# google/nerfactor

Hardware: AMD Instinct MI355X
Metric: rays/sec (NeRF coarse+fine render, 64+128 samples/ray) (higher is better)
Workload: dtype bf16; 1 GPU; lego_3072-shaped NeRF coarse+fine MLP render, 800x800 rays/view, 64+128 samples (BASELINE.json configs[1]); rays_per_view=640000, n_samples_coarse=64, n_samples_fine=128, kernel_variant=7

## Files before the change

### include/nfx.h

```cpp
#ifndef NFX_H_
#define NFX_H_

#include <stddef.h>
#include <stdint.h>

#ifdef __cplusplus
extern "C" {
#endif

#if defined(__GNUC__)
#define NFX_API __attribute__((visibility("default")))
#else
#define NFX_API
#endif

#define NFX_OK 0
#define NFX_EINVAL (-1)
#define NFX_EALIGN (-2)
#define NFX_EHIP (-3)
#define NFX_ENOSUP (-4)

#define NFX_PREC_BF16 0
#define NFX_PREC_FP32 1
#define NFX_PREC_FP32_NATIVE 2
// ... 199 lines not shown
    float *ga, *gb;
    int d;
    float w;
    int kind;
    int flags;
} nfx_loss_term;
NFX_API int nfx_pair_loss_fwd(const nfx_loss_term *terms, int n_terms, const float *dev_alpha, float bg, int64_t n,
                      float *dev_loss, void *stream);
NFX_API int nfx_pair_loss_bwd(const nfx_loss_term *terms, int n_terms, const float *dev_alpha, float bg, int64_t n,
                      const float *dev_dloss, void *stream);


NFX_API int nfx_nerf_sigma_fwd(const float *dev_rayo, const float *dev_rayd, const float *dev_z, int64_t n_rays,
                       int n_samples, const void *dev_geom_blob, int prec, float *dev_sigma, void *stream);

NFX_API size_t nfx_nerf_geom_packed_bytes(int prec);
NFX_API int nfx_nerf_pack_geom_weights(const float *const kernels[12], const float *const biases[12], int prec,
                               void *blob, size_t blob_bytes);
NFX_API int nfx_nerf_sigma_grad(const float *dev_rayo, const float *dev_rayd, const float *dev_z, int64_t n_rays,
                        int n_samples, const void *dev_geom_blob, int prec, float *dev_normal_sigma,
                        void *stream);

NFX_API size_t nfx_nerf_sigma_grad_workspace_bytes(int64_t n_rays, int n_samples);
NFX_API int nfx_nerf_sigma_grad_rows(const float *dev_rayo, const float *dev_rayd, const float *dev_z, int64_t n_rays,
                             int n_samples, const void *dev_geom_blob, int prec, float *dev_normal_sigma,
                             void *dev_workspace, size_t workspace_bytes, void *stream);

NFX_API int nfx_nerf_refine_select(const float *dev_rgbs, const float *dev_z, const float *dev_rayd, int64_t n_rays,
                           int n_samples, float t_min, float a_lo, float a_hi, float sigma_margin, int dilate,
                           int *dev_list, int *dev_count, void *stream);
NFX_API int nfx_nerf_sigma_refine(const float *dev_rayo, const float *dev_rayd, const float *dev_z, int64_t n_rays,
                          int n_samples, const void *dev_geom_blob_fp32, const int *dev_list, const int *dev_count,
                          float *dev_rgbs, void *stream);

#define NFX_OCCGRID_MAX_RES 1024
#define NFX_OCCGRID_MAX_PROBES (1ll << 30)
NFX_API int nfx_nerf_sigma_fwd_list(const float *dev_rayo, const float *dev_rayd, const float *dev_z, int64_t n_rays,
                            int n_samples, const void *dev_geom_blob, int prec, const int *dev_list,
                            const int *dev_count, float *dev_sigma, void *stream);
NFX_API size_t nfx_occgrid_workspace_bytes(int64_t n_rays, int n_samples);
NFX_API int nfx_occgrid_select(const float *dev_rayo, const float *dev_rayd, const float *dev_z, int64_t n_rays,
                       int n_samples, const uint32_t *dev_bits, int res, const float *box, const float *bbox,
                       float *dev_sigma, void *dev_workspace, size_t workspace_bytes, void *stream);
NFX_API int nfx_occgrid_bake(const float *dev_probe_sigma, int res, int probes, float margin, int dilate,
                     uint32_t *dev_bits, uint32_t *dev_workspace, void *stream);


NFX_API int nfx_selftest_mfma_bf16(const float *dev_a, const float *dev_b, float *dev_d, void *stream);
NFX_API int nfx_mlp_generic_split_hilo(void *dev_blob, int d_in, int n_layers, const int *widths, const int *skip_input,
                                       int train, void *stream);
NFX_API size_t nfx_mlp_generic_packed_bytes(int d_in, int n_layers, const int *widths, const int *skip_input, int prec);
NFX_API int nfx_mlp_generic_pack(const float *const *kernels, const float *const *biases, int d_in, int n_layers,
                                 const int *widths, const int *skip_input, int prec, void *blob, size_t blob_bytes);
NFX_API int nfx_mlp_generic_fwd(const float *dev_x, int64_t n, int ld_x, int d_in, int n_layers, const int *widths,
                                const int *acts, const int *skip_input, const void *dev_blob, int prec, float *dev_y,
                                int ld_y, int col0, void *stream);
NFX_API size_t nfx_mlp_generic_train_packed_bytes(int d_in, int n_layers, const int *widths, const int *skip_input,
                                                  int prec);
NFX_API int nfx_mlp_generic_pack_train(const float *const *kernels, const float *const *biases, int d_in, int n_layers,
                                       const int *widths, const int *skip_input, int prec, void *blob,
                                       size_t blob_bytes);
NFX_API size_t nfx_mlp_generic_bwd_workspace_bytes(int64_t n, int d_in, int n_layers, const int *widths,
                                                   const int *skip_input, int prec);
NFX_API int nfx_mlp_generic_bwd(const float *dev_x, int64_t n, int ld_x, int d_in, int n_layers, const int *widths,
                                const int *acts, const int *skip_input, const void *dev_train_blob, int prec,
                                const float *dev_dy, int ld_dy, int col0_dy, float *dev_dx, int ld_dx,
// ... 15 lines not shown
```

### nerfactor_amd/_capi.py

```python
import ctypes
import os

import torch

_HERE = os.path.dirname(os.path.abspath(__file__))
LIB_PATH = os.path.join(_HERE, 'libnfx.so')
if os.environ.get('NFX_LIB_PATH'):
    LIB_PATH = os.environ['NFX_LIB_PATH']

PREC_BF16, PREC_FP32, PREC_FP32_NATIVE = 0, 1, 2
ACT_NONE, ACT_RELU, ACT_SIGMOID, ACT_SOFTPLUS = 0, 1, 2, 3
IN_XYZ, IN_XYZ_LDIR, IN_Z_RUSINK = 0, 1, 2

if not os.path.exists(LIB_PATH):
    raise ImportError(
        "%s not found: build it with `python -m nerfactor_amd.build` (or __graft_entry__.build()); "
        "nerfactor_amd has no fallback path." % LIB_PATH)

lib = ctypes.CDLL(LIB_PATH)

_p = ctypes.c_void_p
_i = ctypes.c_int
_i64 = ctypes.c_int64
_f = ctypes.c_float
# ... 38 lines not shown
    'nfx_composite_bwd': (_i, [_p, _p, _p, _p, _i64, _i, _i, _p, _p, _p]),
    'nfx_nerf_train_packed_bytes': (_sz, [_i]),
    'nfx_nerf_pack_train_weights': (_i, [_pp, _pp, _i, _p, _sz]),
    'nfx_nerf_bwd_workspace_bytes': (_sz, [_i64, _i]),
    'nfx_nerf_mlp_bwd': (_i, [_p, _p, _p, _i64, _i, _p, _i, _p, _p, _sz, _pp, _pp, _p]),
    'nfx_brdf_train_packed_bytes': (_sz, []),
    'nfx_brdf_pack_train_weights': (_i, [_pp, _pp, _i, _i, _p, _sz]),
    'nfx_brdf_spec_bwd_workspace_bytes': (_sz, [_i, _i64]),
    'nfx_brdf_spec_bwd': (_i, [_p, _p, _p, _p, _i, _p, _i, _p, _i, _i64, _p, _p, _p, _p, _sz, _p]),
    'nfx_brdf_spec_bwd_list_bytes': (_sz, [_i64, _i]),
    'nfx_brdf_spec_bwd_rows': (_i, [_p, _p, _p, _p, _i, _p, _i, _p, _i, _i64, _p, _p, _p, _p, _sz, _p, _sz, _p]),
    'nfx_brdf_rows_fwd': (_i, [_p, _i, _p, _i64, _i, _p, _i, _p, _p]),
    'nfx_brdf_rows_bwd_workspace_bytes': (_sz, [_i, _i64, _i]),
    'nfx_brdf_rows_bwd': (_i, [_p, _i, _p, _i64, _i, _p, _i, _p, _p, _sz, _p, _pp, _pp, _p]),
    'nfx_shade_bwd_workspace_bytes': (_sz, [_i]),
    'nfx_shade_bwd': (_i, [_p, _p, _p, _p, _p, _p, _f, _f, _p, _p, _p, _p, _i64, _i, _i, _p, _p, _p, _p, _p, _p,
                           _p, _p, _sz, _p]),
    'nfx_l2_normalize_rows': (_i, [_p, _p, _i64, _i, _f, _p]),
    'nfx_l2_normalize_rows_bwd': (_i, [_p, _p, _p, _i64, _i, _f, _p]),
    'nfx_light_smoothness': (_i, [_p, _i, _i, _f, _f, _p, _p, _p]),
    'nfx_pair_loss_fwd': (_i, [_p, _i, _p, _f, _i64, _p, _p]),
    'nfx_pair_loss_bwd': (_i, [_p, _i, _p, _f, _i64, _p, _p]),
    'nfx_pack_gather': (_i, [_p, _p, _i64, _p, _p]),
    'nfx_amsgrad_step': (_i, [_p, _p, _p, _p, _p, _i64, _f, _f, _f, _f, _i64, _p]),
    'nfx_amsgrad_step_size': (_f, [_f, _f, _f, _i64]),
    'nfx_amsgrad_step_dev': (_i, [_p, _p, _p, _p, _p, _i64, _p, _f, _f, _f, _p]),
    'nfx_nerf_sigma_fwd': (_i, [_p, _p, _p, _i64, _i, _p, _i, _p, _p]),
    'nfx_lvis_fwd_rows': (_i, [_p, _p, _i64, _f, _p, _i, _p, _i, _p, _sz, _p, _p, _p, _p]),
    'nfx_zero_rows': (_i, [_p, _p, _i64, _i, _p]),
    'nfx_shade_fwd_rows': (_i, [_p, _p, _p, _p, _p, _p, _f, _f, _p, _p, _p, _p, _p, _i64, _i, _i, _i, _p, _p]),
    'nfx_shade_olat_fwd_rows': (_i, [_p, _p, _p, _p, _p, _p, _f, _f, _p, _p, _p, _p, _f, _f, _i64, _i, _i, _p, _p, _p, _p]),
    'nfx_nerf_refine_select': (_i, [_p, _p, _p, _i64, _i, _f, _f, _f, _f, _i, _p, _p, _p]),
    'nfx_nerf_sigma_refine': (_i, [_p, _p, _p, _i64, _i, _p, _p, _p, _p, _p]),
    'nfx_nerf_sigma_fwd_list': (_i, [_p, _p, _p, _i64, _i, _p, _i, _p, _p, _p, _p]),
    'nfx_occgrid_workspace_bytes': (_sz, [_i64, _i]),
    'nfx_occgrid_select': (_i, [_p, _p, _p, _i64, _i, _p, _i, _p, _p, _p, _p, _sz, _p]),
    'nfx_occgrid_bake': (_i, [_p, _i, _i, _f, _i, _p, _p, _p]),
    'nfx_nerf_geom_packed_bytes': (_sz, [_i]),
    'nfx_nerf_pack_geom_weights': (_i, [_pp, _pp, _i, _p, _sz]),
    'nfx_nerf_sigma_grad': (_i, [_p, _p, _p, _i64, _i, _p, _i, _p, _p]),
    'nfx_nerf_sigma_grad_workspace_bytes': (_sz, [_i64, _i]),
    'nfx_nerf_sigma_grad_rows': (_i, [_p, _p, _p, _i64, _i, _p, _i, _p, _p, _sz, _p]),
    'nfx_selftest_mfma_bf16': (_i, [_p, _p, _p, _p]),
    'nfx_selftest_sincos': (_i, [_p, _i64, _i, _p, _p]),
    'nfx_selftest_tr16': (_i, [_p, _p, _p, _i, _p]),
    'nfx_mlp_generic_packed_bytes': (_sz, [_i, _i, _p, _p, _i]),
    'nfx_mlp_generic_pack': (_i, [_pp, _pp, _i, _i, _p, _p, _i, _p, _sz]),
    'nfx_mlp_generic_fwd': (_i, [_p, _i64, _i, _i, _i, _p, _p, _p, _p, _i, _p, _i, _i, _p]),
    'nfx_mlp_generic_train_packed_bytes': (_sz, [_i, _i, _p, _p, _i]),
    'nfx_mlp_generic_pack_train': (_i, [_pp, _pp, _i, _i, _p, _p, _i, _p, _sz]),
    'nfx_mlp_generic_bwd_workspace_bytes': (_sz, [_i64, _i, _i, _p, _p, _i]),
    'nfx_mlp_generic_split_hilo': (_i, [_p, _i, _i, _p, _p, _i, _p]),
    'nfx_brdf_rows_geom_fwd': (_i, [_p, _p, _p, _p, _i, _p, _i, _i64, _i, _p, _i, _p, _p]),
    'nfx_brdf_rows_geom_bwd': (_i, [_p, _p, _p, _i, _p, _i, _i64, _i, _p, _i, _p, _p, _p]),
    'nfx_embed_bwd': (_i, [_p, _i64, _i, _i, _p, _i, _i, _p, _p]),
    'nfx_mlp_generic_bwd': (_i, [_p, _i64, _i, _i, _i, _p, _p, _p, _p, _i, _p, _i, _i, _p, _i, _pp, _pp, _p, _sz, _p]),
    'nfx_embed': (_i, [_p, _p, _p, _i64, _i, _i, _i, _i, _p, _i, _i, _p]),
}

for _name, (_res, _args) in SIGNATURES.items():
    _fn = getattr(lib, _name)
    _fn.restype = _res
    _fn.argtypes = _args


class NfxError(RuntimeError):
    """Raised for any non-zero return of the C-ABI; mirrors how the reference surfaces failures as
    Python exceptions (tf.errors.InvalidArgumentError from tf.debugging.*)."""


def last_error():
    buf = ctypes.create_string_buffer(512)
    lib.nfx_last_error(buf, 512)
    return buf.value.decode()


def check(rc, what):
    if rc != 0:
        raise NfxError("%s failed (%d): %s" % (what, rc, last_error()))


OPTION_KEYS = ('nerf_variant', 'nerf_fold', 'nerf_blocks', 'm128_blocks', 'lvis_variant', 'brdf_variant', 'brdf_ct', 'nerf_bwd',
               'nerf_bwd_nw', 'm128_bwd', 'wgrad_lds', 'wgrad_slabs', 'wgrad_rounds', 'wgrad_narrow', 'wgrad_fused', 'lvis_verify', 'lvis_rows', 'brdf_bwd_rows', 'nerf_bwd_rows', 'sigma_grad_rows', 'sigma_variant')


def set_option(key, value):
    check(lib.nfx_set_option(key.encode(), int(value)), 'nfx_set_option(%s)' % key)


def unset_option(key):
    check(lib.nfx_unset_option(key.encode()), 'nfx_unset_option(%s)' % key)


def get_option(key):
    v, isset = _i(0), _i(0)
    check(lib.nfx_get_option(key.encode(), ctypes.byref(v), ctypes.byref(isset)), 'nfx_get_option(%s)' % key)
    return v.value if isset.value else None


class option:

    def __init__(self, key, value):
        self.key, self.value = key, value

    def __enter__(self):
        self.prev = get_option(self.key)
        if self.value is None:
            unset_option(self.key)
        else:
            set_option(self.key, self.value)
        return self

    def __exit__(self, *exc):
        if self.prev is None:
            unset_option(self.key)
        else:
# ... 9 lines not shown
```

### nerfactor_amd/build.py

```python
import fcntl
import os
import subprocess
import sys
from concurrent.futures import ThreadPoolExecutor

HERE = os.path.dirname(os.path.abspath(__file__))
ROOT = os.path.dirname(HERE)
CSRC = os.path.join(HERE, 'csrc')
OBJDIR = os.path.join(ROOT, 'build', 'obj')
LIB = os.path.join(HERE, 'libnfx.so')

HIPCC = os.environ.get('HIPCC', '/opt/rocm/bin/hipcc')
FLAGS = ['--offload-arch=gfx950', '-O3', '-std=c++17', '-ffp-contract=off', '-fPIC', '-fvisibility=hidden',
         '-Wno-unused-result', '-I' + os.path.join(ROOT, 'include')]


VGPR_FORM = ['-mllvm', '-amdgpu-mfma-vgpr-form']
FAST_DIV = ['-fno-hip-fp32-correctly-rounded-divide-sqrt']
PER_FILE_FLAGS = {'lvis_v2.hip': VGPR_FORM, 'nerf_mlp.hip': VGPR_FORM, 'nerf_mlp_v6.hip': VGPR_FORM, 'nerf_sigma_v6.hip': VGPR_FORM,
                  'nerf_geom.hip': VGPR_FORM, 'mlp128_bwd_fused.hip': VGPR_FORM, 'shade.hip': FAST_DIV}


def _sources():
    return sorted(f for f in os.listdir(CSRC) if f.endswith(('.hip', '.cpp')))


def _headers_mtime():
    hs = [os.path.join(CSRC, f) for f in os.listdir(CSRC) if f.endswith('.hpp')]
    hs.append(os.path.join(ROOT, 'include', 'nfx.h'))
    return max(os.path.getmtime(h) for h in hs)


def _job(src, force):
    obj = os.path.join(OBJDIR, src + '.o')
    spath = os.path.join(CSRC, src)
    newest = max(os.path.getmtime(spath), _headers_mtime())
    for line in open(spath):
        if line.startswith('#include "') and line.rstrip().endswith('.hip"'):
            newest = max(newest, os.path.getmtime(os.path.join(CSRC, line.split('"')[1])))
    cmd = [HIPCC] + FLAGS + PER_FILE_FLAGS.get(src, []) + ['-x', 'hip', '-c', spath, '-o', obj]
    stamp = obj + '.cmd'
    same_cmd = os.path.exists(stamp) and open(stamp).read() == ' '.join(cmd)
    return src, obj, cmd, force or not (same_cmd and os.path.exists(obj) and os.path.getmtime(obj) >= newest)


def _compile(job, verbose):
    src, obj, cmd, stale = job
    if not stale:
        return obj, False
    if verbose:
        print(' '.join(cmd), flush=True)
    res = subprocess.run(cmd, stdout=subprocess.PIPE, stderr=subprocess.STDOUT, text=True)
# ... 46 lines not shown
```

### nerfactor_amd/csrc/capi.cpp

```cpp
#include <hip/hip_runtime.h>
#include <stdarg.h>
#include <stdio.h>
#include <stdlib.h>
#include <string.h>

#include <atomic>
#include <vector>

#include "../../include/nfx.h"
#include "nerf_layout.hpp"
#include "nerf_fold_layout.hpp"
#include "pack.hpp"

static thread_local char g_err[512] = "";

int nfx_fail(int code, const char* fmt, ...) {
    va_list ap;
    va_start(ap, fmt);
    vsnprintf(g_err, sizeof(g_err), fmt, ap);
    va_end(ap);
    return code;
}
#define fail nfx_fail
int nfx_hip_result(int e, const char* what);
// ... 27 lines not shown
                         float*, float*, float*, float*, float*, hipStream_t);
int nfx_launch_sample_fine(const float*, const float*, long long, int, int, const float*, float*,
                           hipStream_t);
int nfx_launch_surface(const float*, const float*, const float*, const float*, long long, int, float, int, float*, float*,
                       float*, float*, hipStream_t);
int nfx_launch_selftest_mfma(const float*, const float*, float*, hipStream_t);
int nfx_launch_selftest_sincos(const float*, long long, int, float*, hipStream_t);

int nfx_version(void) { return 100; }

int nfx_last_error(char* buf, size_t len) {
    if (!buf || len == 0) return NFX_EINVAL;
    strncpy(buf, g_err, len - 1);
    buf[len - 1] = 0;
    return NFX_OK;
}

namespace {
struct Option {
    const char* key;
    std::atomic<int> value;
    std::atomic<int> is_set;
};
Option g_options[] = {
    {"nerf_variant", {0}, {0}},
    {"nerf_fold", {0}, {0}},
    {"nerf_blocks", {0}, {0}},
    {"m128_blocks", {0}, {0}},
    {"lvis_variant", {0}, {0}},
    {"lvis_verify", {0}, {0}},
    {"lvis_rows", {0}, {0}},
    {"brdf_bwd_rows", {0}, {0}},
    {"sigma_variant", {0}, {0}},
    {"sigma_grad_rows", {0}, {0}},
    {"nerf_bwd_rows", {0}, {0}},
    {"brdf_variant", {0}, {0}},
    {"brdf_ct", {0}, {0}},
    {"nerf_bwd", {0}, {0}},
    {"nerf_bwd_nw", {0}, {0}},
    {"m128_bwd", {0}, {0}},
    {"wgrad_lds", {0}, {0}},
    {"wgrad_slabs", {0}, {0}},
    {"wgrad_rounds", {0}, {0}},
    {"wgrad_narrow", {0}, {0}},
    {"wgrad_fused", {0}, {0}},
    {"wgrad_splits", {0}, {0}},
    {"wgrad_map", {0}, {0}},
};
Option* find_option(const char* key) {
    if (!key) return nullptr;
    for (Option& o : g_options)
        if (strcmp(o.key, key) == 0) return &o;
    return nullptr;
}
}

int nfx_option_int(const char* key, int dflt) {
    Option* o = find_option(key);
    return o && o->is_set.load(std::memory_order_acquire) ? o->value.load(std::memory_order_relaxed) : dflt;
}
int nfx_set_option(const char* key, int value) {
    Option* o = find_option(key);
    if (!o) return fail(NFX_EINVAL, "nfx_set_option: unknown option '%s'", key ? key : "(null)");
    o->value.store(value, std::memory_order_relaxed);
    o->is_set.store(1, std::memory_order_release);
    return NFX_OK;
// ... 254 lines not shown
```

### nerfactor_amd/csrc/capi_geom.cpp

```cpp
#include <hip/hip_runtime.h>
#include <math.h>
#include <string.h>

#include <vector>

#include "../../include/nfx.h"
#include "nerf_geom_layout.hpp"
#include "pack.hpp"

int nfx_fail(int code, const char* fmt, ...);
int nfx_hip_result(int e, const char* what);
extern "C" int nfx_option_int(const char* name, int dflt);

#define REQUIRE(cond, ...) \
    do {                   \
        if (!(cond)) return nfx_fail(NFX_EINVAL, __VA_ARGS__); \
    } while (0)
#define ALIGNED(p, a) ((((uintptr_t)(p)) & ((a)-1)) == 0)

extern "C" {
int nfx_launch_nerf_sigma_geo(const float*, const float*, const float*, long long, int, const void*, float*, int,
                              hipStream_t);
int nfx_launch_nerf_sigma_grad(const float*, const float*, const float*, long long, int, const void*, float*, int,
                               hipStream_t);
int nfx_launch_refine_select(const float*, const float*, const float*, long long, int, float, float, float, float, int, int*, int*,
                             hipStream_t);
int nfx_launch_nerf_sigma_v6(const float*, const float*, const float*, long long, int, const void*, float*, int, hipStream_t);
int nfx_launch_nerf_sigma_grad_list(const float*, const float*, const float*, long long, int, const void*, float*, const int*,
                                    const int*, int, hipStream_t);
int nfx_launch_nerf_sigma_grad_x3_list(const float*, const float*, const float*, long long, int, const void*, float*,
                                       const int*, const int*, int, hipStream_t);
int nfx_launch_select_density(const float*, long long, float*, void*, hipStream_t);
size_t nfx_nerf_bwd_list_bytes(long long n_pts);
int nfx_launch_nerf_sigma_x3_list(const float*, const float*, const float*, long long, int, const void*, float*, const int*,
                                  const int*, int, hipStream_t);
int nfx_launch_nerf_sigma_x3(const float*, const float*, const float*, long long, int, const void*, float*, int,
                             hipStream_t);
int nfx_launch_nerf_sigma_grad_x3(const float*, const float*, const float*, long long, int, const void*, float*, int,
                                  hipStream_t);
int nfx_launch_nerf_sigma_v6_list(const float*, const float*, const float*, long long, int, const void*, float*, const int*,
                                  const int*, int, hipStream_t);
int nfx_launch_nerf_sigma_x3_list_flat(const float*, const float*, const float*, long long, int, const void*, float*,
                                       const int*, const int*, int, hipStream_t);
size_t nfx_occgrid_list_bytes(long long n_pts);
int nfx_launch_occgrid_select(const float*, const float*, const float*, long long, int, const uint32_t*, int, const float*,
                              const float*, float*, void*, hipStream_t);
int nfx_launch_occgrid_bake(const float*, int, int, float, int, uint32_t*, uint32_t*, hipStream_t);

size_t nfx_nerf_geom_packed_bytes(int prec) {
    using namespace nfx::nerf;
    if (prec == NFX_PREC_BF16) return (size_t)kGeoBlobBytes;
    if (prec == NFX_PREC_FP32) return 2 * (size_t)kGeoWeightBytes + kGeoFloats * sizeof(float);
    return 0;
}
}

static int pack_geom_half(const float* const kernels[12], const float* const biases[12], uint8_t* w0, float* fl) {
    using namespace nfx;
    using namespace nfx::pack;
    std::vector<uint8_t> fwd(nfx_nerf_packed_bytes(NFX_PREC_BF16));
    int rc = nfx_nerf_pack_weights(kernels, biases, NFX_PREC_BF16, fwd.data(), fwd.size());
    if (rc) return rc;
    const size_t enc_bytes = (size_t)nerf::chunk_frag_offset(64) * 1024;
    memcpy(w0, fwd.data(), enc_bytes);
    memcpy(w0 + enc_bytes, fwd.data() + (size_t)nerf::chunk_frag_offset(72) * 1024, 16 * 1024);
    uint8_t* w = w0 + enc_bytes + 16 * 1024;
    std::vector<float> sink(256);
    const Seg hid256{kHidden, 256, 0, nullptr};
    auto hidden_t = [](const float* k) {
        std::vector<float> t((size_t)256 * 256);
        for (int r = 0; r < 256; ++r)
            for (int c = 0; c < 256; ++c) t[(size_t)c * 256 + r] = k[(size_t)r * 256 + c];
        return t;
    };
    auto input_t = [](const float* k, int row0) {
        std::vector<float> t((size_t)256 * 64, 0.f);
// ... 80 lines not shown
        return nfx_hip_result(nfx_launch_nerf_sigma_x3(rayo, rayd, z, (long long)n_rays * n_samples, n_samples, blob,
                                                       sigma, nfx_option_int("nerf_blocks", 256), (hipStream_t)stream),
                              "nerf_sigma_fwd(fp32)");
    return nfx_hip_result(launch_sigma_bf16(rayo, rayd, z, (long long)n_rays * n_samples, n_samples, blob, sigma,
                                            (hipStream_t)stream),
                          "nerf_sigma_fwd");
}

int nfx_nerf_refine_select(const float* rgbs, const float* z, const float* rayd, int64_t n_rays, int n_samples,
                           float t_min, float a_lo, float a_hi, float sigma_margin, int dilate, int* list, int* count,
                           void* stream) {
    REQUIRE(n_rays >= 0 && n_samples >= 1 && n_samples <= 512, "nfx_nerf_refine_select: bad shape (1 <= S <= 512, got %d)", n_samples);
    REQUIRE(n_rays * (int64_t)n_samples < (int64_t)1 << 31, "nfx_nerf_refine_select: %lld samples do not fit int32 indices",
            (long long)(n_rays * n_samples));
    REQUIRE(dilate >= 0 && dilate <= 8, "nfx_nerf_refine_select: dilate = %d (0 .. 8)", dilate);
    REQUIRE(count, "nfx_nerf_refine_select: null count");
    if (n_rays > 0) REQUIRE(rgbs && z && rayd && list, "nfx_nerf_refine_select: null pointer");
    if (n_rays > 0 && !ALIGNED(rgbs, 16)) return nfx_fail(NFX_EALIGN, "nfx_nerf_refine_select: rgbs must be 16-byte aligned");
    return nfx_hip_result(nfx_launch_refine_select(rgbs, z, rayd, (long long)n_rays, n_samples, t_min, a_lo, a_hi, sigma_margin, dilate,
                                                   list, count, (hipStream_t)stream), "nerf_refine_select");
}

int nfx_nerf_sigma_refine(const float* rayo, const float* rayd, const float* z, int64_t n_rays, int n_samples,
                          const void* blob, const int* list, const int* count, float* rgbs, void* stream) {
    REQUIRE(n_rays >= 0 && n_samples >= 1, "nfx_nerf_sigma_refine: bad shape");
    if (n_rays == 0) return NFX_OK;
    REQUIRE(rayo && rayd && z && blob && list && count && rgbs, "nfx_nerf_sigma_refine: null pointer");
    if (!ALIGNED(blob, 16)) return nfx_fail(NFX_EALIGN, "nfx_nerf_sigma_refine: blob must be 16-byte aligned");
    return nfx_hip_result(nfx_launch_nerf_sigma_x3_list(rayo, rayd, z, (long long)n_rays * n_samples, n_samples, blob, rgbs,
                                                        list, count, nfx_option_int("nerf_blocks", 256),
                                                        (hipStream_t)stream), "nerf_sigma_refine");
}

int nfx_nerf_sigma_grad(const float* rayo, const float* rayd, const float* z, int64_t n_rays, int n_samples,
                        const void* geom_blob, int prec, float* normal_sigma, void* stream) {
    REQUIRE(n_rays >= 0 && n_samples >= 1, "nfx_nerf_sigma_grad: bad shape");
    REQUIRE(prec == NFX_PREC_BF16 || prec == NFX_PREC_FP32, "nfx_nerf_sigma_grad: bad prec %d", prec);
    if (n_rays == 0) return NFX_OK;
    REQUIRE(rayo && rayd && z && geom_blob && normal_sigma, "nfx_nerf_sigma_grad: null pointer");
    if (!ALIGNED(geom_blob, 16) || !ALIGNED(normal_sigma, 16))
        return nfx_fail(NFX_EALIGN, "nfx_nerf_sigma_grad: blob and output must be 16-byte aligned");
    if (prec == NFX_PREC_FP32)
        return nfx_hip_result(nfx_launch_nerf_sigma_grad_x3(rayo, rayd, z, (long long)n_rays * n_samples, n_samples,
                                                            geom_blob, normal_sigma,
                                                            nfx_option_int("nerf_blocks", 256), (hipStream_t)stream),
                              "nerf_sigma_grad(fp32)");
    return nfx_hip_result(nfx_launch_nerf_sigma_grad(rayo, rayd, z, (long long)n_rays * n_samples, n_samples,
                                                     geom_blob, normal_sigma, nfx_option_int("nerf_blocks", 256),
                                                     (hipStream_t)stream),
                          "nerf_sigma_grad");
}

static size_t sigma_grad_sigma_bytes(long long n_pts) { return ((size_t)n_pts * 4 + 15) / 16 * 16; }
size_t nfx_nerf_sigma_grad_workspace_bytes(int64_t n_rays, int n_samples) {
    if (n_rays <= 0 || n_samples <= 0) return 0;
    const long long n_pts = (long long)n_rays * n_samples;
    return sigma_grad_sigma_bytes(n_pts) + nfx_nerf_bwd_list_bytes(n_pts);
}

int nfx_nerf_sigma_grad_rows(const float* rayo, const float* rayd, const float* z, int64_t n_rays, int n_samples,
                             const void* geom_blob, int prec, float* normal_sigma, void* workspace,
                             size_t workspace_bytes, void* stream) {
    REQUIRE(n_rays >= 0 && n_samples >= 1, "nfx_nerf_sigma_grad_rows: bad shape");
    REQUIRE(prec == NFX_PREC_BF16 || prec == NFX_PREC_FP32, "nfx_nerf_sigma_grad_rows: bad prec %d", prec);
    if (n_rays == 0) return NFX_OK;
    REQUIRE(rayo && rayd && z && geom_blob && normal_sigma && workspace, "nfx_nerf_sigma_grad_rows: null pointer");
// ... 89 lines not shown
```

### nerfactor_amd/csrc/nerf_geom_x3.hip

```cpp
#include "feat_store.hpp"
#include "mlp_x3.hpp"
#include "nerf_geom_layout.hpp"

namespace nfx {
namespace geo3 {

using x3::Pair;
constexpr int kNW = x3::kNW;
constexpr int kRows = kNW * 32;
constexpr int kZeroTile = nerf::kGeoFloats;
constexpr int kLds = 2 * x3::kSlot + (nerf::kGeoFloats + 32) * 4;
constexpr int kNLD = 4;

template <int KS1, int KS2, int NL_SELF, int NL_NEXT, int KS1A, int KS2A>
__device__ __forceinline__ void fwd_layer(x3::Stream& st, int tid, const float* bias, const Pair (&b1)[KS1A],
                                          const Pair (&b2)[KS2A], Pair (&bout)[16], unsigned (&m)[4]) {
    static_for<0, 8>([&](auto T) {
        constexpr int t = decltype(T)::value;
        f32x16 acc;
        x3::tile<KS1, KS2, (t == 7 ? NL_NEXT : NL_SELF)>(st, tid, bias + 32 * t, b1, b2, acc);
        const unsigned bits = bwd::relu_bits16(acc);
        if constexpr (t & 1) m[t >> 1] |= bits << 16;
        else m[t >> 1] = bits;
        x3::acc_to_pair<true>(acc, bout[2 * t], bout[2 * t + 1]);
    });
}

__device__ __forceinline__ void put(Pair (&dst)[16], int t, int r, float v) {
    __bf16 a, b;
    x3::split(v, a, b);
    dst[2 * t + (r >> 3)].hi[r & 7] = a;
    dst[2 * t + (r >> 3)].lo[r & 7] = b;
}

__device__ __forceinline__ void dgrad(x3::Stream& st, int tid, const float* zero, const Pair (&dz)[16],
                                      const unsigned (&m)[4], Pair (&dout)[16]) {
    static_for<0, 8>([&](auto T) {
        constexpr int t = decltype(T)::value;
        f32x16 acc;
        x3::tile<16, 0, kNLD>(st, tid, zero, dz, dz, acc);
#pragma unroll
        for (int r = 0; r < 16; ++r) put(dout, t, r, bwd::mask_bit(m, t, r) ? acc[r] : 0.f);
    });
}

template <int NL_LAST>
__device__ __forceinline__ void input_grad(x3::Stream& st, int tid, const float* zero, const Pair (&dz)[16],
                                           f32x16 (&dpe)[2]) {
    static_for<0, 2>([&](auto T) {
        constexpr int t = decltype(T)::value;
        f32x16 acc;
        x3::tile<16, 0, (t == 1 ? NL_LAST : kNLD)>(st, tid, zero, dz, dz, acc);
#pragma unroll
        for (int r = 0; r < 16; ++r) dpe[t][r] += acc[r];
    });
}

template <bool GRAD>
__global__ __launch_bounds__(kNW * 64, 1) void nerf_sigma_x3_kernel(
    const float* __restrict__ rayo, const float* __restrict__ rayd, const float* __restrict__ zbuf, long long n_pts,
    int n_samples, const char* __restrict__ blob, float* __restrict__ out, const int* __restrict__ list,
    const int* __restrict__ count, int list_stride) {
    extern __shared__ __attribute__((aligned(16))) char smem[];
    using namespace nerf;
    if (list != nullptr) {
        n_pts = *count;
        if ((long long)blockIdx.x * kRows >= n_pts) return;
    }
    const int tid = threadIdx.x, lane = tid & 63, wave = tid >> 6, h = lane >> 5, p = lane & 31;
    float* fl = reinterpret_cast<float*>(smem + 2 * x3::kSlot);
    {
        const float* src = reinterpret_cast<const float*>(blob + 2 * (size_t)kGeoWeightBytes);
        for (int i = tid; i < kGeoFloats; i += kNW * 64) fl[i] = src[i];
        if (tid < 32) fl[kZeroTile + tid] = 0.f;
    }
    const float* zero = fl + kZeroTile;
    x3::Stream st;
    st.base = reinterpret_cast<const u32x4*>(blob);
    st.end = reinterpret_cast<const u32x4*>(blob + (GRAD ? (size_t)kGeoWeightBytes : (size_t)kGeoFwdFrags * kFragBytes));
    st.ghi = st.base;
    st.lo_off = kGeoWeightBytes / 16;
    st.ring = smem;
    x3::prologue<kNL0>(st, tid);
    const long long n_tiles = (n_pts + kRows - 1) / kRows;
    for (long long tile = blockIdx.x; tile < n_tiles; tile += gridDim.x) {
        const long long row = tile * kRows + wave * 32 + p;
        const bool valid = row < n_pts;
        long long mm = valid ? row : n_pts - 1;
        if (list != nullptr) mm = list[mm];
        float x[3];
        {
            const long long ray = mm / n_samples;
            const float zz = zbuf[mm];
#pragma unroll
            for (int k = 0; k < 3; ++k) x[k] = rayo[ray * 3 + k] + rayd[ray * 3 + k] * zz;
        }
        Pair pe[4];
        x3::posenc_pair<10>(x, h, pe);
        unsigned mk[8][4];
        Pair ha[16], hb[16];
        fwd_layer<4, 0, kNL0, kNLH>(st, tid, fl + 256 * 0, pe, pe, ha, mk[0]);
        fwd_layer<16, 0, kNLH, kNLH>(st, tid, fl + 256 * 1, ha, pe, hb, mk[1]);
        fwd_layer<16, 0, kNLH, kNLH>(st, tid, fl + 256 * 2, hb, pe, ha, mk[2]);
        fwd_layer<16, 0, kNLH, kNLH>(st, tid, fl + 256 * 3, ha, pe, hb, mk[3]);
        fwd_layer<16, 0, kNLH, kNL5>(st, tid, fl + 256 * 4, hb, pe, ha, mk[4]);
        fwd_layer<16, 4, kNL5, kNLH>(st, tid, fl + 256 * 5, ha, pe, hb, mk[5]);
        fwd_layer<16, 0, kNLH, kNLH>(st, tid, fl + 256 * 6, hb, pe, ha, mk[6]);
        fwd_layer<16, 0, kNLH, kNLH>(st, tid, fl + 256 * 7, ha, pe, hb, mk[7]);
        float sigma;
        {
            f32x16 acc;
            x3::tile<16, 0, (GRAD ? kNLD : kNL0)>(st, tid, fl + kGeoBiasSig, hb, pe, acc);
            sigma = acc[0];
        }
        if constexpr (!GRAD) {
            if (valid && h == 0) {
                if (list != nullptr) out[list_stride * (mm + 1) - 1] = sigma;
                else out[row] = sigma;
            }
        } else {
#pragma unroll
            for (int t = 0; t < 8; ++t)
#pragma unroll
                for (int r = 0; r < 16; ++r) {
                    const float wv = fl[kGeoWSig + 32 * t + (r & 3) + 8 * (r >> 2) + 4 * h];
                    put(ha, t, r, bwd::mask_bit(mk[7], t, r) ? wv : 0.f);
                }
            f32x16 dpe[2];
#pragma unroll
            for (int t = 0; t < 2; ++t)
#pragma unroll
                for (int r = 0; r < 16; ++r) dpe[t][r] = 0.f;
            dgrad(st, tid, zero, ha, mk[6], hb);
            dgrad(st, tid, zero, hb, mk[5], ha);
            input_grad<kNLD>(st, tid, zero, ha, dpe);
            dgrad(st, tid, zero, ha, mk[4], hb);
            dgrad(st, tid, zero, hb, mk[3], ha);
            dgrad(st, tid, zero, ha, mk[2], hb);
            dgrad(st, tid, zero, hb, mk[1], ha);
            dgrad(st, tid, zero, ha, mk[0], hb);
            input_grad<kNL0>(st, tid, zero, hb, dpe);
            float g[3] = {0.f, 0.f, 0.f};
#pragma unroll
            for (int q = 0; q < 32; ++q) {
                const float dq = dpe[q >> 4][q & 15];
                if (q < 30) {
                    const float freq = (float)(1 << (q / 3));
                    const float other = sin_shifted(x[q % 3] * freq, h ^ 1);
                    g[q % 3] += dq * freq * (h ? -other : other);
                } else if (q == 30) {
                    if (h) g[2] += dq; else g[0] += dq;
                } else {
                    if (!h) g[1] += dq;
                }
            }
#pragma unroll
            for (int k = 0; k < 3; ++k) g[k] += __shfl_xor(g[k], 32, 64);
            if (valid && h == 0) {
                const float on = sigma > 0.f ? 1.f : 0.f;
                const float gx = g[0] * on, gy = g[1] * on, gz = g[2] * on;
                const float inv = -1.0f / sqrtf(fmaxf(gx * gx + gy * gy + gz * gz, 1e-12f));
                reinterpret_cast<float4*>(out)[list != nullptr ? mm : row] = make_float4(gx * inv, gy * inv, gz * inv, sigma);
            }
        }
    }
}

template <bool GRAD>
static int launch(const float* rayo, const float* rayd, const float* z, long long n_pts, int n_samples,
                  const void* blob, float* out, int max_blocks, hipStream_t st, const int* list = nullptr,
                  const int* count = nullptr, int list_stride = 4) {
    if (n_pts <= 0) return 0;
    const long long tiles = (n_pts + kRows - 1) / kRows;
    const int grid = (int)(tiles < max_blocks ? tiles : max_blocks);
    auto k = nerf_sigma_x3_kernel<GRAD>;
    hipError_t e = hipFuncSetAttribute(reinterpret_cast<const void*>(k), hipFuncAttributeMaxDynamicSharedMemorySize, kLds);
    if (e != hipSuccess) return (int)e;
    hipLaunchKernelGGL(k, dim3(grid), dim3(kNW * 64), kLds, st, rayo, rayd, z, n_pts, n_samples, (const char*)blob, out,
                       list, count, list_stride);
    return (int)hipGetLastError();
}

}
}

extern "C" int nfx_launch_nerf_sigma_grad_x3(const float* rayo, const float* rayd, const float* z, long long n_pts,
                                             int n_samples, const void* blob, float* out, int max_blocks,
                                             hipStream_t st) {
    return nfx::geo3::launch<true>(rayo, rayd, z, n_pts, n_samples, blob, out, max_blocks, st);
}
extern "C" int nfx_launch_nerf_sigma_x3(const float* rayo, const float* rayd, const float* z, long long n_pts,
                                        int n_samples, const void* blob, float* out, int max_blocks, hipStream_t st) {
    return nfx::geo3::launch<false>(rayo, rayd, z, n_pts, n_samples, blob, out, max_blocks, st);
}
extern "C" int nfx_launch_nerf_sigma_grad_x3_list(const float* rayo, const float* rayd, const float* z, long long n_pts,
                                                  int n_samples, const void* blob, float* out, const int* list,
                                                  const int* count, int max_blocks, hipStream_t st) {
    return nfx::geo3::launch<true>(rayo, rayd, z, n_pts, n_samples, blob, out, max_blocks, st, list, count);
}
extern "C" int nfx_launch_nerf_sigma_x3_list(const float* rayo, const float* rayd, const float* z, long long n_pts,
                                             int n_samples, const void* blob, float* rgbs, const int* list,
                                             const int* count, int max_blocks, hipStream_t st) {
    return nfx::geo3::launch<false>(rayo, rayd, z, n_pts, n_samples, blob, rgbs, max_blocks, st, list, count);
}
extern "C" int nfx_launch_nerf_sigma_x3_list_flat(const float* rayo, const float* rayd, const float* z, long long n_pts,
                                                  int n_samples, const void* blob, float* out, const int* list,
                                                  const int* count, int max_blocks, hipStream_t st) {
    return nfx::geo3::launch<false>(rayo, rayd, z, n_pts, n_samples, blob, out, max_blocks, st, list, count, 1);
}
```

### nerfactor_amd/ops.py

```python
import ctypes
import os

import numpy as np
import torch

from . import _capi
from ._capi import PREC_BF16, PREC_FP32, PREC_FP32_NATIVE, check, lib

_PREC = {'bf16': PREC_BF16, 'fp32': PREC_FP32, 'fp32_native': PREC_FP32_NATIVE, PREC_BF16: PREC_BF16, PREC_FP32: PREC_FP32,
         PREC_FP32_NATIVE: PREC_FP32_NATIVE}
_ACT = {None: 0, 'none': 0, 'relu': 1, 'sigmoid': 2, 'softplus': 3}


def _ptr(t):
    return None if t is None else ctypes.c_void_p(t.data_ptr())


def _stream():
    return ctypes.c_void_p(torch.cuda.current_stream().cuda_stream)


def _dev(t, name, shape=None):
    if t is None:
        return None
# ... 793 lines not shown
            first = ws_bytes // 4 - nerf_bwd_list_words((hi - lo) * s)[3]
            NERF_BWD_STATS.append((ws.view(torch.int32)[first:first + 1].clone(), (hi - lo) * s))
    return ws


def pack_nerf_geom_weights(kernels, biases, prec='bf16'):
    if len(kernels) != 12 or len(biases) != 12:
        raise _capi.NfxError("pack_nerf_geom_weights: need 12 kernels and 12 biases")
    return _pack(lib.nfx_nerf_geom_packed_bytes, lib.nfx_nerf_pack_geom_weights, kernels, biases, (_PREC[prec],))


def _ray_args(rayo, rayd, z, blob):
    rayo = _dev(rayo, 'rayo', (None, 3))
    n = rayo.shape[0]
    rayd = _dev(rayd, 'rayd', (n, 3))
    z = _dev(z, 'z', (n, None))
    if not blob.is_cuda or blob.dtype != torch.uint8:
        raise _capi.NfxError("blob must be a CUDA uint8 tensor")
    return rayo, rayd, z, n, z.shape[1]


def nerf_sigma_fwd(rayo, rayd, z, blob, prec='bf16'):
    rayo, rayd, z, n, s = _ray_args(rayo, rayd, z, blob)
    out = torch.empty((n, s), dtype=torch.float32, device=z.device)
    check(lib.nfx_nerf_sigma_fwd(_ptr(rayo), _ptr(rayd), _ptr(z), n, s, _ptr(blob), _PREC[prec], _ptr(out),
                                 _stream()), 'nfx_nerf_sigma_fwd')
    return out


def nerf_refine_last_sample(rayo, rayd, z, rgbs, geom_blob_fp32):
    n, s = z.shape
    if n == 0 or s < 2:
        return rgbs
    sig = nerf_sigma_fwd(rayo, rayd, z[:, -1:].contiguous(), geom_blob_fp32, 'fp32')
    rgbs[:, -1, 3] = sig[:, 0]
    return rgbs


REFINE_T_MIN, REFINE_A_LO, REFINE_A_HI, REFINE_DILATE = 1e-3, 1e-3, 0.999, 0
REFINE_MARGIN_FACTOR = 2.


def nerf_refine_coarse(rayo, rayd, z, rgbs, geom_blob_fp32, t_min=REFINE_T_MIN, a_lo=REFINE_A_LO, a_hi=REFINE_A_HI,
                       dilate=REFINE_DILATE, sigma_margin=0., want_count=False):
    rayo, rayd, z, n, s = _ray_args(rayo, rayd, z, geom_blob_fp32)
    if not (isinstance(rgbs, torch.Tensor) and rgbs.is_contiguous()):
        raise _capi.NfxError("nerf_refine_coarse: rgbs is updated in place and must be contiguous")
    rgbs = _dev(rgbs, 'rgbs', (n, s, 4))
    count = torch.empty(1, dtype=torch.int32, device=z.device)
    if n == 0 or s < 2:
        count.zero_()
        return (rgbs, count) if want_count else rgbs
    lst = torch.empty(n * s, dtype=torch.int32, device=z.device)
    check(lib.nfx_nerf_refine_select(_ptr(rgbs), _ptr(z), _ptr(rayd), n, s, t_min, a_lo, a_hi, sigma_margin, dilate, _ptr(lst), _ptr(count),
                                     _stream()), 'nfx_nerf_refine_select')
    check(lib.nfx_nerf_sigma_refine(_ptr(rayo), _ptr(rayd), _ptr(z), n, s, _ptr(geom_blob_fp32), _ptr(lst), _ptr(count),
                                    _ptr(rgbs), _stream()), 'nfx_nerf_sigma_refine')
    return (rgbs, count) if want_count else rgbs


def nerf_coarse_error(rayo, rayd, z, rgbs, geom_blob_fp32, max_rays=4096, q=0.999, geom_blob_bf16=None):
    n = min(int(z.shape[0]), max_rays)
    if n == 0 or z.shape[1] < 2:
        return 0., 0.
    step = max(1, int(z.shape[0]) // n)
    pick = slice(0, n * step, step)
    o, d, zz = rayo[pick].contiguous(), rayd[pick].contiguous(), z[pick].contiguous()
    s32 = nerf_sigma_fwd(o, d, zz, geom_blob_fp32, 'fp32')
# ... 240 lines not shown
```

Measured before the change: 4.723 million rays/s.

## Add pipelined fp32 sigma kernel with weight DMA ring and fused last-sample refine

Adds a new non-grad sigma kernel that streams weight chunks into a three-slot LDS ring via DMA two chunks ahead. It also prefetches A fragments and overlaps each tile's ReLU/split epilogue and next bias load with the following tile's MFMAs. This kernel becomes the default for all non-grad x3 sigma launches. Separately, the last-sample refine now indexes the final sample directly and writes sigma into rgbs in place, instead of making a contiguous z slice, running a separate output and scattering it. The cost is extra code complexity and more barriers per tile.

```diff
diff --git a/include/nfx.h b/include/nfx.h
--- a/include/nfx.h
+++ b/include/nfx.h
@@ -255,6 +255,9 @@
 NFX_API int nfx_nerf_sigma_refine(const float *dev_rayo, const float *dev_rayd, const float *dev_z, int64_t n_rays,
                           int n_samples, const void *dev_geom_blob_fp32, const int *dev_list, const int *dev_count,
                           float *dev_rgbs, void *stream);
+
+NFX_API int nfx_nerf_sigma_refine_last(const float *dev_rayo, const float *dev_rayd, const float *dev_z, int64_t n_rays,
+                               int n_samples, const void *dev_geom_blob_fp32, float *dev_rgbs, void *stream);
 
 #define NFX_OCCGRID_MAX_RES 1024
 #define NFX_OCCGRID_MAX_PROBES (1ll << 30)
diff --git a/nerfactor_amd/_capi.py b/nerfactor_amd/_capi.py
--- a/nerfactor_amd/_capi.py
+++ b/nerfactor_amd/_capi.py
@@ -94,6 +94,7 @@
     'nfx_shade_olat_fwd_rows': (_i, [_p, _p, _p, _p, _p, _p, _f, _f, _p, _p, _p, _p, _f, _f, _i64, _i, _i, _p, _p, _p, _p]),
     'nfx_nerf_refine_select': (_i, [_p, _p, _p, _i64, _i, _f, _f, _f, _f, _i, _p, _p, _p]),
     'nfx_nerf_sigma_refine': (_i, [_p, _p, _p, _i64, _i, _p, _p, _p, _p, _p]),
+    'nfx_nerf_sigma_refine_last': (_i, [_p, _p, _p, _i64, _i, _p, _p, _p]),
     'nfx_nerf_sigma_fwd_list': (_i, [_p, _p, _p, _i64, _i, _p, _i, _p, _p, _p, _p]),
     'nfx_occgrid_workspace_bytes': (_sz, [_i64, _i]),
     'nfx_occgrid_select': (_i, [_p, _p, _p, _i64, _i, _p, _i, _p, _p, _p, _p, _sz, _p]),
@@ -143,7 +144,8 @@
 
 
 OPTION_KEYS = ('nerf_variant', 'nerf_fold', 'nerf_blocks', 'm128_blocks', 'lvis_variant', 'brdf_variant', 'brdf_ct', 'nerf_bwd',
-               'nerf_bwd_nw', 'm128_bwd', 'wgrad_lds', 'wgrad_slabs', 'wgrad_rounds', 'wgrad_narrow', 'wgrad_fused', 'lvis_verify', 'lvis_rows', 'brdf_bwd_rows', 'nerf_bwd_rows', 'sigma_grad_rows', 'sigma_variant')
+               'nerf_bwd_nw', 'm128_bwd', 'wgrad_lds', 'wgrad_slabs', 'wgrad_rounds', 'wgrad_narrow', 'wgrad_fused', 'lvis_verify', 'lvis_rows', 'brdf_bwd_rows', 'nerf_bwd_rows', 'sigma_grad_rows', 'sigma_variant',
+               'sigma_x3_variant')
 
 
 def set_option(key, value):
diff --git a/nerfactor_amd/build.py b/nerfactor_amd/build.py
--- a/nerfactor_amd/build.py
+++ b/nerfactor_amd/build.py
@@ -18,6 +18,7 @@
 VGPR_FORM = ['-mllvm', '-amdgpu-mfma-vgpr-form']
 FAST_DIV = ['-fno-hip-fp32-correctly-rounded-divide-sqrt']
 PER_FILE_FLAGS = {'lvis_v2.hip': VGPR_FORM, 'nerf_mlp.hip': VGPR_FORM, 'nerf_mlp_v6.hip': VGPR_FORM, 'nerf_sigma_v6.hip': VGPR_FORM,
+                  'nerf_sigma_x3_pipe.hip': VGPR_FORM,
                   'nerf_geom.hip': VGPR_FORM, 'mlp128_bwd_fused.hip': VGPR_FORM, 'shade.hip': FAST_DIV}
 
 
diff --git a/nerfactor_amd/csrc/capi.cpp b/nerfactor_amd/csrc/capi.cpp
--- a/nerfactor_amd/csrc/capi.cpp
+++ b/nerfactor_amd/csrc/capi.cpp
@@ -83,6 +83,7 @@
     {"lvis_rows", {0}, {0}},
     {"brdf_bwd_rows", {0}, {0}},
     {"sigma_variant", {0}, {0}},
+    {"sigma_x3_variant", {0}, {0}},
     {"sigma_grad_rows", {0}, {0}},
     {"nerf_bwd_rows", {0}, {0}},
     {"brdf_variant", {0}, {0}},
diff --git a/nerfactor_amd/csrc/capi_geom.cpp b/nerfactor_amd/csrc/capi_geom.cpp
--- a/nerfactor_amd/csrc/capi_geom.cpp
+++ b/nerfactor_amd/csrc/capi_geom.cpp
@@ -42,6 +42,8 @@
                                   const int*, int, hipStream_t);
 int nfx_launch_nerf_sigma_x3_list_flat(const float*, const float*, const float*, long long, int, const void*, float*,
                                        const int*, const int*, int, hipStream_t);
+int nfx_launch_nerf_sigma_x3_last(const float*, const float*, const float*, long long, int, const void*, float*, int,
+                                  hipStream_t);
 size_t nfx_occgrid_list_bytes(long long n_pts);
 int nfx_launch_occgrid_select(const float*, const float*, const float*, long long, int, const uint32_t*, int, const float*,
                               const float*, float*, void*, hipStream_t);
@@ -188,6 +190,17 @@
                                                         (hipStream_t)stream), "nerf_sigma_refine");
 }
 
+int nfx_nerf_sigma_refine_last(const float* rayo, const float* rayd, const float* z, int64_t n_rays, int n_samples,
+                               const void* blob, float* rgbs, void* stream) {
+    REQUIRE(n_rays >= 0 && n_samples >= 1, "nfx_nerf_sigma_refine_last: bad shape");
+    if (n_rays == 0) return NFX_OK;
+    REQUIRE(rayo && rayd && z && blob && rgbs, "nfx_nerf_sigma_refine_last: null pointer");
+    if (!ALIGNED(blob, 16)) return nfx_fail(NFX_EALIGN, "nfx_nerf_sigma_refine_last: blob must be 16-byte aligned");
+    return nfx_hip_result(nfx_launch_nerf_sigma_x3_last(rayo, rayd, z, (long long)n_rays, n_samples, blob, rgbs,
+                                                        nfx_option_int("nerf_blocks", 256), (hipStream_t)stream),
+                          "nerf_sigma_refine_last");
+}
+
 int nfx_nerf_sigma_grad(const float* rayo, const float* rayd, const float* z, int64_t n_rays, int n_samples,
                         const void* geom_blob, int prec, float* normal_sigma, void* stream) {
     REQUIRE(n_rays >= 0 && n_samples >= 1, "nfx_nerf_sigma_grad: bad shape");
diff --git a/nerfactor_amd/csrc/nerf_geom_x3.hip b/nerfactor_amd/csrc/nerf_geom_x3.hip
--- a/nerfactor_amd/csrc/nerf_geom_x3.hip
+++ b/nerfactor_amd/csrc/nerf_geom_x3.hip
@@ -1,6 +1,10 @@
 #include "feat_store.hpp"
 #include "mlp_x3.hpp"
 #include "nerf_geom_layout.hpp"
+
+extern "C" int nfx_option_int(const char* name, int dflt);
+extern "C" int nfx_launch_nerf_sigma_x3_pipe(const float*, const float*, const float*, long long, int, const void*, float*,
+                                             const int*, const int*, int, int, int, hipStream_t);
 
 namespace nfx {
 namespace geo3 {
@@ -60,7 +64,7 @@
 __global__ __launch_bounds__(kNW * 64, 1) void nerf_sigma_x3_kernel(
     const float* __restrict__ rayo, const float* __restrict__ rayd, const float* __restrict__ zbuf, long long n_pts,
     int n_samples, const char* __restrict__ blob, float* __restrict__ out, const int* __restrict__ list,
-    const int* __restrict__ count, int list_stride) {
+    const int* __restrict__ count, int list_stride, int last_sample) {
     extern __shared__ __attribute__((aligned(16))) char smem[];
     using namespace nerf;
     if (list != nullptr) {
@@ -88,6 +92,7 @@
         const bool valid = row < n_pts;
         long long mm = valid ? row : n_pts - 1;
         if (list != nullptr) mm = list[mm];
+        else if (!GRAD && last_sample) mm = (mm + 1) * n_samples - 1;
         float x[3];
         {
             const long long ray = mm / n_samples;
@@ -115,7 +120,7 @@
         }
         if constexpr (!GRAD) {
             if (valid && h == 0) {
-                if (list != nullptr) out[list_stride * (mm + 1) - 1] = sigma;
+                if (list != nullptr || last_sample) out[list_stride * (mm + 1) - 1] = sigma;
                 else out[row] = sigma;
             }
         } else {
@@ -169,15 +174,18 @@
 template <bool GRAD>
 static int launch(const float* rayo, const float* rayd, const float* z, long long n_pts, int n_samples,
                   const void* blob, float* out, int max_blocks, hipStream_t st, const int* list = nullptr,
-                  const int* count = nullptr, int list_stride = 4) {
+                  const int* count = nullptr, int list_stride = 4, int last_sample = 0) {
     if (n_pts <= 0) return 0;
+    if (!GRAD && nfx_option_int("sigma_x3_variant", 1) != 0)
+        return nfx_launch_nerf_sigma_x3_pipe(rayo, rayd, z, n_pts, n_samples, blob, out, list, count, list_stride, last_sample,
+                                             max_blocks, st);
     const long long tiles = (n_pts + kRows - 1) / kRows;
     const int grid = (int)(tiles < max_blocks ? tiles : max_blocks);
     auto k = nerf_sigma_x3_kernel<GRAD>;
     hipError_t e = hipFuncSetAttribute(reinterpret_cast<const void*>(k), hipFuncAttributeMaxDynamicSharedMemorySize, kLds);
     if (e != hipSuccess) return (int)e;
     hipLaunchKernelGGL(k, dim3(grid), dim3(kNW * 64), kLds, st, rayo, rayd, z, n_pts, n_samples, (const char*)blob, out,
-                       list, count, list_stride);
+                       list, count, list_stride, last_sample);
     return (int)hipGetLastError();
 }
 
@@ -208,3 +216,7 @@
                                                   const int* count, int max_blocks, hipStream_t st) {
     return nfx::geo3::launch<false>(rayo, rayd, z, n_pts, n_samples, blob, out, max_blocks, st, list, count, 1);
 }
+extern "C" int nfx_launch_nerf_sigma_x3_last(const float* rayo, const float* rayd, const float* z, long long n_rays,
+                                             int n_samples, const void* blob, float* rgbs, int max_blocks, hipStream_t st) {
+    return nfx::geo3::launch<false>(rayo, rayd, z, n_rays, n_samples, blob, rgbs, max_blocks, st, nullptr, nullptr, 4, 1);
+}
diff --git a/nerfactor_amd/csrc/nerf_sigma_x3_pipe.hip b/nerfactor_amd/csrc/nerf_sigma_x3_pipe.hip
--- /dev/null
+++ b/nerfactor_amd/csrc/nerf_sigma_x3_pipe.hip
@@ -0,0 +1,217 @@
+#include "mlp_x3.hpp"
+#include "lds_dma.hpp"
+#include "nerf_geom_layout.hpp"
+
+namespace nfx {
+namespace geo3p {
+
+using x3::Pair;
+constexpr int kNW = x3::kNW;
+constexpr int kRows = kNW * 32;
+constexpr int kRing = 3;
+constexpr int kDist = 2;
+constexpr int kPreA = 3;
+constexpr int kABuf = kPreA + 1;
+constexpr int kNChunks = 65;
+constexpr int kSeq = 66;
+constexpr int kLds = kRing * x3::kSlot + nerf::kGeoFloats * 4;
+static_assert(kSeq % kRing == 0, "the chunk sequence wraps on the ring");
+static_assert(kLds <= 160 * 1024, "LDS");
+
+constexpr int slot_of(int k) { return k % kRing; }
+constexpr int used_frags(int k) { return k < 8 ? 4 : k < 40 ? 16 : k < 48 ? 20 : 16; }
+constexpr int bias_of(int k) { return k < 64 ? 32 * k : nerf::kGeoBiasSig; }
+static_assert(used_frags(0) % kABuf == 0 && used_frags(8) % kABuf == 0 && used_frags(40) % kABuf == 0,
+              "the A-pair buffer carries across tiles");
+
+struct Ctx {
+    char* smem;
+    const char* blob;
+    unsigned smem_lds;
+    int wave;
+    int lane;
+};
+
+template <int K>
+__device__ __forceinline__ void dma_chunk(const Ctx& cx) {
+    constexpr int n = used_frags(K) / kNW;
+    unsigned long long base = reinterpret_cast<unsigned long long>(cx.blob);
+    unsigned lds = cx.smem_lds;
+    asm volatile("" : "+s"(base), "+s"(lds));
+    const char* g = reinterpret_cast<const char*>(base) + (size_t)nerf::chunk_frag_offset(K) * kFragBytes + cx.wave * (n * 1024);
+    const unsigned l = lds + slot_of(K) * x3::kSlot + cx.wave * (n * 1024);
+    lds_dma_pieces<n>(cx.lane * 16, g, l);
+    lds_dma_pieces<n>(cx.lane * 16, g + nerf::kGeoWeightBytes, l + kSlotBytes);
+}
+
+template <int K, int E>
+__device__ __forceinline__ void read_a(const Ctx& cx, Pair (&ab)[kABuf]) {
+    constexpr int KS = used_frags(K);
+    constexpr int C = E < KS ? K : K + 1, F = E < KS ? E : E - KS;
+    if constexpr (C < kNChunks) {
+        const char* f = cx.smem + slot_of(C) * x3::kSlot + F * kFragBytes + cx.lane * 16;
+        ab[E % kABuf].hi = *reinterpret_cast<const bf16x8*>(f);
+        ab[E % kABuf].lo = *reinterpret_cast<const bf16x8*>(f + kSlotBytes);
+    }
+}
+
+__device__ __forceinline__ void bias_to_acc(const float* bias_tile, int lane, f32x16& acc) {
+    const float* bt = bias_tile + 4 * (lane >> 5);
+#pragma unroll
+    for (int g = 0; g < 4; ++g) {
+        const f32x4 v = *reinterpret_cast<const f32x4*>(bt + 8 * g);
+        acc[4 * g + 0] = v[0];
+        acc[4 * g + 1] = v[1];
+        acc[4 * g + 2] = v[2];
+        acc[4 * g + 3] = v[3];
+    }
+}
+
+__device__ __forceinline__ void relu_split2(float v0, float v1, Pair& dst, int j) {
+    v0 = __builtin_amdgcn_fmed3f(v0, 0.0f, __builtin_inff());
+    v1 = __builtin_amdgcn_fmed3f(v1, 0.0f, __builtin_inff());
+    const f32x2 v = {v0, v1};
+    const bf16x2 hi = __builtin_convertvector(v, bf16x2);
+    const f32x2 back = __builtin_convertvector(hi, f32x2);
+    const bf16x2 lo = __builtin_convertvector(v - back, bf16x2);
+    dst.hi[j] = hi[0];
+    dst.hi[j + 1] = hi[1];
+    dst.lo[j] = lo[0];
+    dst.lo[j + 1] = lo[1];
+}
+
+struct EpiPair {
+    const f32x16& acc;
+    Pair& lo8;
+    Pair& hi8;
+    template <int R0, int R1>
+    __device__ __forceinline__ void run() {
+#pragma unroll
+        for (int r = R0; r < R1; r += 2) {
+            if (r < 8) relu_split2(acc[r], acc[r + 1], lo8, r);
+            else relu_split2(acc[r], acc[r + 1], hi8, r - 8);
+        }
+    }
+};
+struct EpiNone {
+    template <int R0, int R1>
+    __device__ __forceinline__ void run() {}
+};
+
+template <int K, int KS1, int KS2, int KS1A, int KS2A, typename Epi>
+__device__ __forceinline__ void tile(const Ctx& cx, const float* fl, const Pair (&b1)[KS1A], const Pair (&b2)[KS2A],
+                                     f32x16& acc, f32x16& acc_next, Pair (&ab)[kABuf], Epi&& prev) {
+    constexpr int KS = KS1 + KS2;
+    static_assert(KS == used_frags(K), "k-steps of the chunk");
+    constexpr int PIECES = KS >= 16 ? 8 : 4;
+    constexpr int SP = PIECES < KS ? PIECES : KS - 1;
+    constexpr int K2 = (K + kDist) % kSeq;
+    if constexpr (K2 < kNChunks) dma_chunk<K2>(cx);
+    static_for<0, KS>([&](auto S) {
+        constexpr int s = decltype(S)::value;
+        read_a<K, s + kPreA>(cx, ab);
+        const Pair& a = ab[s % kABuf];
+        const Pair& b = s < KS1 ? b1[s < KS1 ? s : 0] : b2[s >= KS1 ? s - KS1 : 0];
+        acc = __builtin_amdgcn_mfma_f32_32x32x16_bf16(a.lo, b.hi, acc, 0, 0, 0);
+        acc = __builtin_amdgcn_mfma_f32_32x32x16_bf16(a.hi, b.lo, acc, 0, 0, 0);
+        acc = __builtin_amdgcn_mfma_f32_32x32x16_bf16(a.hi, b.hi, acc, 0, 0, 0);
+        if constexpr (s < PIECES) prev.template run<16 * s / PIECES, 16 * (s + 1) / PIECES>();
+        if constexpr (s == SP && K + 1 < kNChunks) bias_to_acc(fl + bias_of(K + 1), cx.lane, acc_next);
+    });
+    asm volatile("s_waitcnt vmcnt(0) lgkmcnt(0)\n\ts_barrier" ::: "memory");
+}
+
+template <int K0, int KS1, int KS2, int KS1A, int KS2A, typename Epi0>
+__device__ __forceinline__ void layer(const Ctx& cx, const float* fl, const Pair (&b1)[KS1A], const Pair (&b2)[KS2A],
+                                      Pair (&bout)[16], f32x16 (&accs)[2], Pair (&ab)[kABuf], Epi0&& prev0) {
+    static_for<0, 8>([&](auto T) {
+        constexpr int t = decltype(T)::value;
+        constexpr int K = K0 + t;
+        if constexpr (t == 0) {
+            tile<K, KS1, KS2>(cx, fl, b1, b2, accs[K & 1], accs[(K + 1) & 1], ab, prev0);
+        } else {
+            EpiPair e{accs[(K - 1) & 1], bout[2 * (t - 1)], bout[2 * (t - 1) + 1]};
+            tile<K, KS1, KS2>(cx, fl, b1, b2, accs[K & 1], accs[(K + 1) & 1], ab, e);
+        }
+    });
+}
+
+__global__ __launch_bounds__(kNW * 64, 1) void nerf_sigma_x3_pipe_kernel(
+    const float* __restrict__ rayo, const float* __restrict__ rayd, const float* __restrict__ zbuf, long long n_pts,
+    int n_samples, const char* __restrict__ blob, float* __restrict__ out, const int* __restrict__ list,
+    const int* __restrict__ count, int list_stride, int last_sample) {
+    extern __shared__ __attribute__((aligned(16))) char smem[];
+    using namespace nerf;
+    if (list != nullptr) {
+        n_pts = *count;
+        if ((long long)blockIdx.x * kRows >= n_pts) return;
+    }
+    const int tid = threadIdx.x, lane = tid & 63, wave = tid >> 6, h = lane >> 5, p = lane & 31;
+    float* fl = reinterpret_cast<float*>(smem + kRing * x3::kSlot);
+    {
+        const float* src = reinterpret_cast<const float*>(blob + 2 * (size_t)kGeoWeightBytes);
+        for (int i = tid; i < kGeoFloats; i += kNW * 64) fl[i] = src[i];
+    }
+    typedef __attribute__((address_space(3))) char lds_char;
+    const Ctx cx{smem, blob, (unsigned)__builtin_amdgcn_readfirstlane((unsigned)(uintptr_t)(lds_char*)smem),
+                 __builtin_amdgcn_readfirstlane(wave), lane};
+    dma_chunk<0>(cx);
+    const bool indirect = list != nullptr || last_sample != 0;
+    const long long n_tiles = (n_pts + kRows - 1) / kRows;
+    for (long long tl = blockIdx.x; tl < n_tiles; tl += gridDim.x) {
+        dma_chunk<1>(cx);
+        const long long row = tl * kRows + wave * 32 + p;
+        const bool valid = row < n_pts;
+        long long mm = valid ? row : n_pts - 1;
+        if (list != nullptr) mm = list[mm];
+        else if (last_sample) mm = (mm + 1) * n_samples - 1;
+        float x[3];
+        {
+            const long long ray = mm / n_samples;
+            const float zz = zbuf[mm];
+#pragma unroll
+            for (int k = 0; k < 3; ++k) x[k] = rayo[ray * 3 + k] + rayd[ray * 3 + k] * zz;
+        }
+        Pair pe[4];
+        x3::posenc_pair<10>(x, h, pe);
+        asm volatile("s_waitcnt vmcnt(0) lgkmcnt(0)\n\ts_barrier" ::: "memory");
+        f32x16 accs[2];
+        Pair ab[kABuf];
+        bias_to_acc(fl, lane, accs[0]);
+        static_for<0, kPreA>([&](auto E) { read_a<0, decltype(E)::value>(cx, ab); });
+        Pair ha[16], hb[16];
+        auto pend = [&](Pair& lo8, Pair& hi8) { return EpiPair{accs[1], lo8, hi8}; };
+        layer<0, 4, 0>(cx, fl, pe, pe, ha, accs, ab, EpiNone{});
+        layer<8, 16, 0>(cx, fl, ha, pe, hb, accs, ab, pend(ha[14], ha[15]));
+        layer<16, 16, 0>(cx, fl, hb, pe, ha, accs, ab, pend(hb[14], hb[15]));
+        layer<24, 16, 0>(cx, fl, ha, pe, hb, accs, ab, pend(ha[14], ha[15]));
+        layer<32, 16, 0>(cx, fl, hb, pe, ha, accs, ab, pend(hb[14], hb[15]));
+        layer<40, 16, 4>(cx, fl, ha, pe, hb, accs, ab, pend(ha[14], ha[15]));
+        layer<48, 16, 0>(cx, fl, hb, pe, ha, accs, ab, pend(hb[14], hb[15]));
+        layer<56, 16, 0>(cx, fl, ha, pe, hb, accs, ab, pend(ha[14], ha[15]));
+        tile<64, 16, 0>(cx, fl, hb, pe, accs[0], accs[1], ab, pend(hb[14], hb[15]));
+        const float sigma = accs[0][0];
+        if (valid && h == 0) {
+            if (indirect) out[list_stride * (mm + 1) - 1] = sigma;
+            else out[row] = sigma;
+        }
+    }
+}
+
+}
+}
+
+extern "C" int nfx_launch_nerf_sigma_x3_pipe(const float* rayo, const float* rayd, const float* z, long long n_pts,
+                                             int n_samples, const void* blob, float* out, const int* list, const int* count,
+                                             int list_stride, int last_sample, int max_blocks, hipStream_t st) {
+    using namespace nfx::geo3p;
+    if (n_pts <= 0) return 0;
+    const long long tiles = (n_pts + kRows - 1) / kRows;
+    const int grid = (int)(tiles < max_blocks ? tiles : max_blocks);
+    hipError_t e = hipFuncSetAttribute(reinterpret_cast<const void*>(nerf_sigma_x3_pipe_kernel),
+                                       hipFuncAttributeMaxDynamicSharedMemorySize, kLds);
+    if (e != hipSuccess) return (int)e;
+    hipLaunchKernelGGL(nerf_sigma_x3_pipe_kernel, dim3(grid), dim3(kNW * 64), kLds, st, rayo, rayd, z, n_pts, n_samples,
+                       (const char*)blob, out, list, count, list_stride, last_sample);
+    return (int)hipGetLastError();
+}
diff --git a/nerfactor_amd/ops.py b/nerfactor_amd/ops.py
--- a/nerfactor_amd/ops.py
+++ b/nerfactor_amd/ops.py
@@ -849,8 +849,11 @@
     n, s = z.shape
     if n == 0 or s < 2:
         return rgbs
-    sig = nerf_sigma_fwd(rayo, rayd, z[:, -1:].contiguous(), geom_blob_fp32, 'fp32')
-    rgbs[:, -1, 3] = sig[:, 0]
+    if not (isinstance(rgbs, torch.Tensor) and rgbs.is_contiguous()):
+        raise _capi.NfxError("nerf_refine_last_sample: rgbs is updated in place and must be contiguous")
+    rayo, rayd, z, n, s = _ray_args(rayo, rayd, z, geom_blob_fp32)
+    check(lib.nfx_nerf_sigma_refine_last(_ptr(rayo), _ptr(rayd), _ptr(z), n, s, _ptr(geom_blob_fp32),
+                                         _ptr(_dev(rgbs, 'rgbs', (n, s, 4))), _stream()), 'nfx_nerf_sigma_refine_last')
     return rgbs
 
 
```

Measured after the change: 4.787 million rays/s (median of 6 runs). +1.4%, better.
